# franioli/icepy4d

Measured on AMD Instinct MI355X. Metric: matched stereo image-pairs/sec (4096 kpts, 1080p), higher is better.
Workload: dtype f32

## Files before the change

### icepy4d_amd/_lib.py

```python
from __future__ import annotations

import ctypes as C
import os
import subprocess
from typing import Optional

_HERE = os.path.dirname(os.path.abspath(__file__))
CSRC = os.path.join(_HERE, "csrc")
LIB_PATH = os.environ.get("ICEMATCH_LIB") or os.path.join(CSRC, "libicematch.so")

_lib: Optional[C.CDLL] = None


class IcematchError(RuntimeError):

    def __init__(self, what: str, rc: int, message: str):
        super().__init__(f"{what} failed ({rc}): {message}")
        self.what, self.rc = what, rc


class LightGlueConf(C.Structure):
    _fields_ = [("depth_confidence", C.c_double), ("width_confidence", C.c_double),
                ("filter_threshold", C.c_double), ("n_layers", C.c_int), ("pruning_min_kpts", C.c_int)]


class SuperGlueConf(C.Structure):
    _fields_ = [("sinkhorn_iterations", C.c_int), ("match_threshold", C.c_double), ("n_layers", C.c_int)]


_P = C.c_void_p
_I = C.c_int
_F = C.c_float
_D = C.c_double
_L = C.c_longlong

SIGNATURES = {
    "im_version": [],
    "im_ctx_create": [_I, C.POINTER(_P)],
    "im_ctx_destroy": [_P],
    "im_last_error": [_P],
    "im_ctx_reserve": [_P, _I, _I, _I, _I],
    "im_profile_begin": [_P],
    "im_profile_end": [_P, C.c_char_p, C.c_size_t],
    "im_set_tensor": [_P, C.c_char_p, C.c_char_p, _P, C.c_size_t],
    "im_finalize_weights": [_P, C.c_char_p],
    "im_superpoint_forward": [_P, _P, _I, _I, _I, _I, _I, _F, _I, _I, _I, _P, _P, _P, _P, _P],
    "im_superpoint_candidates": [_P, _I, _P, _P],
    "im_lightglue_forward": [_P, _P, _P, _P, _P, C.POINTER(LightGlueConf), _P, _P, _P, _P, _P],
    "im_lightglue_forward_pairs": [_P, _I, _P, _P, _P, _P, C.POINTER(LightGlueConf), _P, _P, _P, _P, _P],
    "im_pack_records": [_P, _I, _P, _P, _P, _P, _I, _P, _P, _P],
    "im_superglue_forward": [_P, _P, _P, _P, _P, _P, C.POINTER(SuperGlueConf), _P, _P, _P, _P],
    "im_pack_record": [_P, _P, _P, _P, _P, _I, _P, _P],
    "im_debug_read": [_P, C.c_char_p, _P, C.c_size_t, _P],
    "im_debug_clock_probe": [_P, _I, _P, _P],
    "im_debug_guard_failures": [],
    "im_debug_guard_selftest": [_P, _P],
    "im_debug_guards_check": [_P, _P],
    "im_pyr_down": [_P, _P, _P, _I, _I, _I, _I, _P],
    "im_pyr_up": [_P, _P, _P, _I, _I, _I, _I, _P],
    "im_gemm_nt": [_P, _P, _P, _P, _P, _I, _I, _I, _F, _I, _P],
    "im_ffn_fused": [_P, _I, _P, _P, _P, _P, _P, _P, _P, _P, _I, _I, _P, _P],
    "im_conv3x3": [_P, _P, _P, _P, _P, _I, _I, _I, _I, _I, _I, _I, _P],
    "im_conv3x3_winograd": [_P, _P, _P, _P, _P, _I, _I, _I, _I, _I, _I, _I, _P],
    "im_flash_attn": [_P, _P, _P, _P, _P, _P, _I, _I, _I, _I, _F, _P],
    "im_nms": [_P, _P, _P, _I, _I, _I, _I, _P],
    "im_select_topk": [_P, _P, _I, _I, _I, _I, _F, _I, _P, _P, _P, _P],
    "im_sample_descriptors": [_P, _P, _I, _I, _I, _P, _P, _P, _P],
    "im_assign_from_sim": [_P, _P, _I, _I, _I, _P, _P, _F, _P, _P, _P, _P, _P],
    "im_log_optimal_transport": [_P, _P, _I, _I, _I, _F, _I, _P, _P],
    "im_merge_tile_matches": [_P, _I, _I, _P, _P, _P, _P, _P, _P, _P, _P, _P, _P, _P, _P],
    "im_gather_rows": [_P, _P, _I, _P, _I, _P, _P],
    "im_ransac_fundamental": [_P, _P, _P, _I, _I, C.c_double, C.c_uint, _P, _P, _P, _P],
    "im_ransac_essential": [_P, _P, _P, _I, _I, C.c_double, C.c_uint, _P, _P, _P, _P],
    "im_triangulate_linear": [_P, _P, _P, _P, _P, _I, _P, _P],
    "im_forient": [_P, _P, _I, _I, _I, _I, _P, _P],
    "im_template_match_oc": [_P, _P, _I, _I, _P, _I, _I, _I, _P, _P, _I, _I, _I, _I, _P, _P],
    "im_dsm_round": [_P, _P, _L, _F, _P, _P, _P, _P, _P, _P],
    "im_dsm_group_mean": [_P, _P, _P, _P, _P, _P, _P, _L, _P, _P, _P, _P, _P],
    "im_dsm_rasterize": [_P, _P, _P, _P, _P, _P, _L, _P, _P, _I, _P, _I, _D, _D, _D, _D, _D, _P, _P],
    "im_project_colors": [_P, _P, _L, _L, _P, _L, _L, _P, _L, _L, _I, _I, _I, _P, _P, _I, _I, _I, _P, _I, _P, _P, _P, _P],
    "im_undistort_points": [_P, _P, _L, _P, _P, _P],
    "im_triangulate_iterative": [_P, _P, _P, _I, _L, _P, _P, _P, _P, _D, _I, _P, _P, _P, _P, _P],
    "im_triangulate_table": [_P, _P, _I, _I, _P, _I, _I, _D, _I, _L, _P, _P, _P, _P, _P, _P],
    "im_binned_lds_capacity": [],
    "im_binned_cells": [_P, _P, _L, _I, _P, _P, _P, _P, _P, _I, _P, _P],
    "im_binned_stats": [_P, _P, _P, _L, _I, _L, _P, _I, _P, _P, _P],
    "im_tracked_points": [_P, _P, _P, _L, _P, _I, _P, _P, _P, _L, _P, _P, _P, _I, _P, _P, _P, _P, _P],
    "im_undistort_image": [_P, _P, _I, _I, _I, _I, _P, _P, _P],
    "im_warp_perspective": [_P, _P, _I, _I, _I, _I, _P, _I, _I, _P, _P],
    "im_knn_max_cells": [],
    "im_knn_cells": [_P, _P, _L, _P, _I, _I, _I, _P, _P],
    "im_knn_cell_ranges": [_P, _P, _L, _L, _P, _P],
    "im_knn_self": [_P, _P, _P, _P, _L, _P, _I, _I, _I, _I, _D, _P, _P, _P, _P, _P, _P, _P],
    "im_dod_chunk": [],
    "im_dod_max_cells": [],
    "im_dod_max_batch_cells": [],
    "im_dod_bounds": [_P, _P, _P, _I, _I, _P, _P, _P],
    "im_dod_keys": [_P, _P, _P, _I, _P, _I, _I, _D, _P, _P, _P, _P],
    "im_dod_reduce": [_P, _P, _P, _I, _P, _I, _I, _D, _P, _P, _P, _P, _P, _P],
    "im_crop_polygon": [_P, _P, _L, _I, _I, _P, _I, _I, _P, _P, _P, _P],
}


def build(force: bool = False) -> str:
    if force:
        subprocess.run(["make", "-C", CSRC, "clean"], check=True, capture_output=True)
    r = subprocess.run(["make", "-C", CSRC, "-j8"], capture_output=True, text=True)
    if r.returncode != 0:
        raise RuntimeError(f"building libicematch.so failed:\n{r.stdout[-4000:]}\n{r.stderr[-4000:]}")
    return LIB_PATH


def load() -> C.CDLL:
    global _lib
# ... 58 lines not shown
```

### icepy4d_amd/csrc/block.h

```cpp
#pragma once
#include "ctx.h"

namespace im {

struct BlockFfn {
    int act = 0;
    const float* w0 = nullptr; const float* w0p = nullptr;
    const float* b0 = nullptr;
    const float* ln_g = nullptr; const float* ln_b = nullptr;
    const float* w3 = nullptr; const float* w3p = nullptr;
    const float* b3 = nullptr;
    const char* name_fused = nullptr; const char* name_ffn0 = nullptr; const char* name_ffn3 = nullptr;
};

int launch_block_proj(im_ctx* ctx, hipStream_t s, const char* name, const GemmArgs& g, const float* wp_layers, int layer);

int launch_block_tail(im_ctx* ctx, hipStream_t s, const AttnArgs& at, const BlockFfn& f, const GemmArgs& base, float* x);

}
```

### icepy4d_amd/csrc/block.hip

```cpp
#include "block.h"

#include "lg_misc.h"
#include "workspace.h"

namespace im {

int launch_block_proj(im_ctx* ctx, hipStream_t s, const char* name, const GemmArgs& g, const float* wp_layers, int layer) {
    if (env_is_1("IM_PROJ_TILED")) {
        IM_LAUNCH(ctx, name, s, launch_gemm(g, s));
        return 0;
    }
    GemmArgs r = g;
    r.wp = reinterpret_cast<const unsigned char*>(wp_layers) + (size_t)layer * g.N * 256 * 6;
    IM_LAUNCH(ctx, name, s, launch_proj_rows(r, s));
    return 0;
}

int launch_block_tail(im_ctx* ctx, hipStream_t s, const AttnArgs& at, const BlockFfn& f, const GemmArgs& base, float* x) {
    Workspace* ws = ctx->ws;
    const long xb = (long)base.m_max * 256, hb = (long)base.m_max * 512;
    IM_LAUNCH(ctx, "attn_kv_planes", s, launch_attn_planes(at, s));
    IM_LAUNCH(ctx, at.cross ? "flash_attn_cross" : "flash_attn_self", s, launch_flash_attn(at, s));
    static const bool unfused = env_is_1("IM_FFN_UNFUSED");
    if (!unfused) {
        FfnArgs a;
        a.act = f.act; a.x = x; a.x_bstride = xb; a.att = at.out; a.att_bstride = xb;
        a.w0p = f.w0p; a.b0 = f.b0; a.ln_g = f.ln_g; a.ln_b = f.ln_b; a.w3p = f.w3p; a.b3 = f.b3;
        a.m_max = base.m_max; a.batch = base.batch; a.m_ptr = base.m_ptr; a.active = base.active; a.pstride = base.pstride;
        IM_LAUNCH(ctx, f.name_fused, s, launch_ffn_fused(a, s));
        return 0;
    }
    {
        GemmArgs g = base;
        g.A = x; g.a_bstride = xb; g.lda = 256; g.A1 = at.out; g.a1_bstride = xb; g.lda1 = 256; g.ksplit = 256;
        g.W = f.w0; g.ldw = 512; g.bias = f.b0; g.N = 512; g.K = 512;
        g.C = ws->h; g.c_bstride = hb; g.ldc = 512; g.epi = f.act == 1 ? EPI_BIAS_RELU : EPI_BIAS;
        IM_LAUNCH(ctx, f.name_ffn0, s, launch_gemm(g, s));
    }
    if (f.act == 0)
        IM_LAUNCH(ctx, "lg_layernorm_gelu", s, launch_layernorm_gelu(ws->h, hb, ws->st, base.batch, base.m_max, f.ln_g, f.ln_b, s));
    {
        GemmArgs g = base;
        g.A = ws->h; g.a_bstride = hb; g.lda = 512; g.W = f.w3; g.ldw = 512; g.bias = f.b3; g.N = 256; g.K = 512;
        g.C = x; g.c_bstride = xb; g.ldc = 256; g.R = x; g.r_bstride = xb; g.ldr = 256; g.epi = EPI_BIAS_RESID;
        IM_LAUNCH(ctx, f.name_ffn3, s, launch_gemm(g, s));
    }
    return 0;
}

}
```

### icepy4d_amd/csrc/capi.hip

```cpp
#include "ctx.h"
#include "lg_misc.h"
#include "sp_post.h"
#include "workspace.h"

#include <algorithm>
#include <cstdio>
#include <cstdlib>
#include <cstring>

using namespace im;

template <int N, typename F>
static hipError_t with_uploads(const float* const (&src)[N], const size_t (&sizes)[N], hipStream_t st, F&& launch) {
    float* d[N] = {};
    hipError_t e = hipSuccess;
    for (int i = 0; i < N && e == hipSuccess; ++i) {
        e = hipMalloc(&d[i], sizes[i] * sizeof(float));
        if (e == hipSuccess) e = hipMemcpy(d[i], src[i], sizes[i] * sizeof(float), hipMemcpyHostToDevice);
    }
    if (e == hipSuccess) e = launch(d);
    const hipError_t e2 = hipStreamSynchronize(st);
    for (int i = 0; i < N; ++i) hipFree(d[i]);
    return e != hipSuccess ? e : e2;
}
// ... 186 lines not shown
        IM_GROW(ctx, ctx->grow(ctx->scratch.clock[1], bytes, "clock_probe_convolution"), -22, "im_debug_clock_probe: allocation failed");
        IM_HIP(ctx, hipMemsetAsync(ctx->scratch.clock[0].p, 0, bytes, s));
        IM_HIP(ctx, hipMemsetAsync(ctx->scratch.clock[1].p, 0, bytes, s));
        IM_HIP(ctx, hipStreamSynchronize(s));
        ctx->clock_armed = true;
        return 0;
    }
    if (!ctx->scratch.clock[0].p || !h_out) return ctx->fail(-51, "im_debug_clock_probe: not armed");
    std::vector<unsigned long long> h((size_t)CLOCK_PROBE_SLOTS * 2);
    const void* src[2] = {ctx->scratch.clock[0].p, ctx->scratch.clock[1].p};
    for (int c = 0; c < 2; ++c) {
        IM_HIP(ctx, hipMemcpyAsync(h.data(), src[c], bytes, hipMemcpyDeviceToHost, s));
        IM_HIP(ctx, hipStreamSynchronize(s));
        std::vector<double> mhz;
        for (int i = 0; i < CLOCK_PROBE_SLOTS; ++i)
            if (h[2 * i + 1] > 0) mhz.push_back(100.0 * (double)h[2 * i] / (double)h[2 * i + 1]);
        std::sort(mhz.begin(), mhz.end());
        h_out[2 * c] = mhz.empty() ? 0.0 : mhz[mhz.size() / 2];
        h_out[2 * c + 1] = (double)mhz.size();
    }
    if (arm == 0) ctx->clock_armed = false;
    return 0;
}

int im_gemm_nt(im_ctx* ctx, const float* d_a, const float* d_w, const float* d_bias, float* d_c, int m, int n, int k,
               float alpha, int big_tile, void* stream) {
    IM_CHECK_CTX(ctx);
    GemmArgs g;
    g.A = d_a; g.lda = k; g.W = d_w; g.ldw = k; g.bias = d_bias; g.N = n; g.K = k; g.m_max = m;
    g.C = d_c; g.ldc = n; g.alpha = alpha; g.epi = EPI_BIAS; g.big_tile = big_tile & 1; g.bx = (big_tile >> 1) & 1;
    IM_HIP(ctx, launch_gemm(g, (hipStream_t)stream));
    return 0;
}

int im_ffn_fused(im_ctx* ctx, int act, float* d_x, const float* d_att, const float* h_w0, const float* h_b0, const float* h_ln_g,
                   const float* h_ln_b, const float* h_w3, const float* h_b3, int n_images, int n_rows, const int32_t* d_n, void* stream) {
    IM_CHECK_CTX(ctx);
    if (n_images < 1 || n_rows < 1 || act < 0 || act > 1 || (act == 0 && (!h_ln_g || !h_ln_b))) return ctx->fail(-12, "im_ffn_fused: bad arguments");
    if (act == 1) h_ln_g = h_ln_b = h_b0;
    const std::vector<float> p0 = pack_frag_weights(h_w0, 512, 512), p3 = pack_frag_weights(h_w3, 256, 512);
    const size_t sizes[6] = {p0.size(), 512, 512, 512, p3.size(), 256};
    const float* src[6] = {p0.data(), h_b0, h_ln_g, h_ln_b, p3.data(), h_b3};
    hipStream_t st = (hipStream_t)stream;
    IM_HIP(ctx, with_uploads(src, sizes, st, [&](float* const* d) {
        FfnArgs f;
        f.act = act; f.x = d_x; f.x_bstride = (long)n_rows * 256; f.att = d_att; f.att_bstride = (long)n_rows * 256;
        f.w0p = d[0]; f.b0 = d[1]; f.ln_g = d[2]; f.ln_b = d[3]; f.w3p = d[4]; f.b3 = d[5];
        f.m_max = n_rows; f.batch = n_images; f.m_ptr = d_n; f.pstride = 2;
        return ctx->timed("ffn_fused", st, [&] { return launch_ffn_fused(f, st); });
    }));
    return 0;
}

static int conv3x3_entry(im_ctx* ctx, bool wino, const float* d_in, const float* h_weight, const float* h_bias, float* d_out,
                         int b, int h, int w, int cin, int cout, int relu, int pool, void* stream) {
    IM_CHECK_CTX(ctx);
    if (cin % 16 || cout % 64) return ctx->fail(-10, "im_conv3x3: cin %% 16 and cout %% 64 must be 0");
    std::vector<float> packed = wino ? pack_conv3x3_wino(h_weight, cout, cin) : pack_conv3x3(h_weight, cout, cin);
    std::vector<float> planes = wino ? pack_conv3x3_wino_bx(h_weight, cout, cin) : std::vector<float>(1);
    const size_t sizes[3] = {packed.size(), (size_t)cout, planes.size()};
    const float* src[3] = {packed.data(), h_bias, planes.data()};
    hipStream_t st = (hipStream_t)stream;
    IM_HIP(ctx, with_uploads(src, sizes, st, [&](float* const* d) {
        ConvArgs a;
        a.in = d_in; a.w = d[0]; a.bias = d[1]; a.out = d_out; a.B = b; a.H = h; a.W = w; a.Cin = cin; a.Cout = cout;
        a.relu = relu; a.pool = pool;
        if (wino) a.wx = d[2];
        return ctx->timed(wino ? "conv_wino" : "conv_direct", st, [&] { return wino ? launch_conv3x3_wino(a, st) : launch_conv3x3(a, st); });
    }));
    return 0;
}

int im_conv3x3(im_ctx* ctx, const float* d_in, const float* h_weight, const float* h_bias, float* d_out, int b, int h,
               int w, int cin, int cout, int relu, int pool, void* stream) {
    return conv3x3_entry(ctx, false, d_in, h_weight, h_bias, d_out, b, h, w, cin, cout, relu, pool, stream);
}

int im_conv3x3_winograd(im_ctx* ctx, const float* d_in, const float* h_weight, const float* h_bias, float* d_out, int b,
                        int h, int w, int cin, int cout, int relu, int pool, void* stream) {
    return conv3x3_entry(ctx, true, d_in, h_weight, h_bias, d_out, b, h, w, cin, cout, relu, pool, stream);
}

int im_flash_attn(im_ctx* ctx, const float* d_q, const float* d_k, const float* d_v, float* d_out, const int32_t* d_n,
                  int n_max, int batch, int heads, int cross, float scale, void* stream) {
    IM_CHECK_CTX(ctx);
    AttnArgs a;
    a.q = d_q; a.k = d_k; a.v = d_v; a.hstride = (long)n_max * 64; a.bstride = a.hstride * heads;
    a.out = d_out; a.ldo = heads * 64; a.out_bstride = (long)n_max * a.ldo;
    a.n_ptr = d_n; a.n_max = n_max; a.batch = batch; a.heads = heads; a.cross = cross & 1; a.f32_form = (cross >> 1) & 1; a.scale = scale;
    im_ctx::StageScratch& sc = ctx->scratch;
    const bool wants_planes = !(cross & 4) && !a.f32_form;
    IM_GROW(ctx, ctx->grow(sc.attn_part, attn_part_floats(n_max, batch, heads) * sizeof(float), "stage_attn_part"), -11, "im_flash_attn: out of device memory");
    IM_GROW(ctx, ctx->grow(sc.attn_cnt, attn_counter_ints(n_max, batch, heads) * sizeof(int), "stage_attn_cnt", true), -11, "im_flash_attn: out of device memory");
    if (wants_planes) IM_GROW(ctx, ctx->grow(sc.attn_planes, attn_planes_bytes(n_max, batch, heads), "stage_attn_planes"), -11, "im_flash_attn: out of device memory");
    a.part = sc.attn_part.as<float>(); a.counters = sc.attn_cnt.as<int>(); a.planes = wants_planes ? sc.attn_planes.as<unsigned char>() : nullptr;
    IM_HIP(ctx, launch_attn_planes(a, (hipStream_t)stream));
    IM_HIP(ctx, launch_flash_attn(a, (hipStream_t)stream));
    IM_GUARD_CHECK(ctx, (hipStream_t)stream, "im_flash_attn");
    return 0;
}

int im_nms(im_ctx* ctx, const float* d_scores, float* d_out, int n_images, int h, int w, int radius, void* stream) {
    IM_CHECK_CTX(ctx);
    Workspace* ws = ctx->ws;
    if (!ws || (long)n_images * h * w > (long)ws->smap_floats)
        return ctx->fail(-41, "im_nms: exceeds the reserved workspace");
// ... 52 lines not shown
```

### icepy4d_amd/csrc/gemm.hip

```cpp
#include "bf16x3.h"
#include "common.h"
#include "kernels.h"

namespace im {

template <int BM, int BN, int BK, int EPI, bool BX>
__global__ __launch_bounds__(256) void gemm_nt_kernel(GemmArgs a) {
    constexpr int LDS_LD = BK + 4;
    constexpr int WM = BM / 2, WN = BN / 2;
    constexpr int MB = WM / 32, NB = WN / 32;
    constexpr int F4 = BK / 4;
    constexpr int A_IT = BM * F4 / 256, B_IT = BN * F4 / 256;
    constexpr int XS = BK * 2 + 16, XPA = BM * XS, XPB = BN * XS;
    __shared__ __attribute__((aligned(16))) float smem[BX ? 3 * (XPA + XPB) / 4 : (BM + BN) * LDS_LD];
    float* sA = smem;
    float* sB = smem + BM * LDS_LD;
    unsigned char* const xA = reinterpret_cast<unsigned char*>(smem);
    unsigned char* const xB = xA + 3 * XPA;

    const int gm = (a.m_max + BM - 1) / BM;
    const int z = blockIdx.y;
    const int pair = a.pair_batched ? z : (z >> 1);
    if (a.active && a.active[pair * a.pstride] == 0) return;
    const int M = a.m_ptr ? a.m_ptr[a.pair_batched ? z * a.pstride : (z >> 1) * a.pstride + (z & 1)] : a.m_max;
// ... 277 lines not shown
    {                                                                                                                \
        const unsigned char* ap = psm + c * PS + ((kc_) * 16 + hh * 8) * 2;                                          \
        const u32x4 ah = *reinterpret_cast<const u32x4*>(ap), am = *reinterpret_cast<const u32x4*>(ap + PLANE),   \
                     al = *reinterpret_cast<const u32x4*>(ap + 2 * PLANE);                                          \
        acc = mfma_bf(ah, b_[2], acc);                                                                              \
        acc = mfma_bf(al, b_[0], acc);                                                                              \
        acc = mfma_bf(am, b_[1], acc);                                                                              \
        acc = mfma_bf(ah, b_[1], acc);                                                                              \
        acc = mfma_bf(am, b_[0], acc);                                                                              \
        acc = mfma_bf(ah, b_[0], acc);                                                                              \
    }
#pragma unroll 1
    for (int j = 0; j < TILES; ++j) {
        const int tile = j * 8 + wave;
        f32x16 acc;
#pragma unroll
        for (int r = 0; r < 16; ++r) acc[r] = 0.f;
#pragma unroll 1
        for (int kc = 0; kc < 16; kc += 4) {
            const int s_ = j * 16 + kc;
            PR_LOAD(b3, s_ + 3)
            __builtin_amdgcn_sched_barrier(0);
            PR_SIX(b0, kc)
            __builtin_amdgcn_sched_barrier(0);
            PR_LOAD(b0, s_ + 4)
            __builtin_amdgcn_sched_barrier(0);
            PR_SIX(b1, kc + 1)
            __builtin_amdgcn_sched_barrier(0);
            PR_LOAD(b1, s_ + 5)
            __builtin_amdgcn_sched_barrier(0);
            PR_SIX(b2, kc + 2)
            __builtin_amdgcn_sched_barrier(0);
            PR_LOAD(b2, s_ + 6)
            __builtin_amdgcn_sched_barrier(0);
            PR_SIX(b3, kc + 3)
            __builtin_amdgcn_sched_barrier(0);
        }
        P_STAMP(2 + 2 * j)
        const int colbase = tile * 32;
        const int col = colbase + c;
        const float bv = a.bias ? a.bias[col] : 0.f;
        const unsigned rowl = m0 + 4 * hh;
        const int which = colbase >> 8, hd = colbase & 255;
        float* dst = a.q;
        if constexpr (EPI == EPI_QKV_ROPE) dst = which == 0 ? a.q : (which == 1 ? a.k : a.v);
        if constexpr (EPI == EPI_HEADS_QV) dst = which ? a.v : a.q;
        const __amdgpu_buffer_rsrc_t rD = make_rsrc(dst + (long)z * a.head_bstride + (long)(hd >> 6) * a.head_stride, (unsigned)M * 256u);
        const int d = (hd & 63) + c;
        const unsigned vo = (rowl * 64 + d) * 4u;
        float scale = a.alpha;
        if constexpr (EPI == EPI_QKV_ROPE) scale = 1.f;
        if constexpr (EPI == EPI_HEADS_QV) scale = which ? 1.f : a.alpha;
        const bool rope = EPI == EPI_QKV_ROPE && which < 2 && a.cs;
        if (rope) {
            const __amdgpu_buffer_rsrc_t rCs = make_rsrc(a.cs + (long)z * a.enc_bstride, (unsigned)M * 128u);
            const __amdgpu_buffer_rsrc_t rSn = make_rsrc(a.sn + (long)z * a.enc_bstride, (unsigned)M * 128u);
            const unsigned ve = (rowl * 32 + (d >> 1)) * 4u;
#pragma unroll
            for (int r = 0; r < 16; ++r) {
                const unsigned so = ((r & 3) + 8 * (r >> 2)) * 128u;
                const float cs = __uint_as_float(__builtin_amdgcn_raw_buffer_load_b32(rCs, ve, so, 0));
                const float sn = __uint_as_float(__builtin_amdgcn_raw_buffer_load_b32(rSn, ve, so, 0));
                const float val = acc[r] + bv;
                const float partner = __shfl_xor(val, 1);
                const float outv = (d & 1) ? (val * cs) + (partner * sn) : (val * cs) + ((-partner) * sn);
                __builtin_amdgcn_raw_buffer_store_b32(__float_as_uint(outv), rD, vo, ((r & 3) + 8 * (r >> 2)) * 256u, 0);
            }
        } else {
#pragma unroll
            for (int r = 0; r < 16; ++r)
                __builtin_amdgcn_raw_buffer_store_b32(__float_as_uint(scale * (acc[r] + bv)), rD, vo, ((r & 3) + 8 * (r >> 2)) * 256u, 0);
        }
        P_STAMP(3 + 2 * j)
    }
#undef PR_LOAD
#undef PR_SIX
}

template <int EPI, int TILES>
static hipError_t launch_proj_rows_t(const GemmArgs& a, hipStream_t s) {
    const dim3 grid((a.m_max + pr::BM - 1) / pr::BM, a.batch), block(pr::NT);
    return launch_dyn_lds<proj_rows_kernel<EPI, TILES>>(grid, block, pr::LDS_BYTES, s, a);
}

hipError_t launch_proj_rows(const GemmArgs& a, hipStream_t s) {
    if (!a.wp || a.K != 256 || a.lda != 256 || a.A1 || a.sel || a.w_bstride || a.n_ptr || a.pair_batched) return hipErrorInvalidValue;
    if (a.m_max <= 0 || a.batch <= 0) return hipSuccess;
    if (a.epi == EPI_QKV_ROPE && a.N == 768) return launch_proj_rows_t<EPI_QKV_ROPE, 3>(a, s);
    if (a.epi == EPI_HEADS_QV && a.N == 512) return launch_proj_rows_t<EPI_HEADS_QV, 2>(a, s);
    return hipErrorInvalidValue;
}

hipError_t launch_gemm(const GemmArgs& a, hipStream_t s) {
    if (a.K % 32 != 0 || (a.A1 && a.ksplit % 64 != 0)) return hipErrorInvalidValue;
    const int bm = a.big_tile ? 128 : 64, bn = bm;
    dim3 grid(((a.N + bn - 1) / bn) * ((a.m_max + bm - 1) / bm), a.batch), block(256);
    if (grid.x == 0) return hipSuccess;
#define IM_GEMM_CASE(E)                                                                  \
    case E:                                                                              \
        if (a.bx) {                                                                      \
            if (a.big_tile) hipLaunchKernelGGL((gemm_nt_kernel<128, 128, 32, E, true>), grid, block, 0, s, a);   \
            else hipLaunchKernelGGL((gemm_nt_kernel<64, 64, 32, E, true>), grid, block, 0, s, a);               \
        } else {                                                                         \
            if (a.big_tile) hipLaunchKernelGGL((gemm_nt_kernel<128, 128, 32, E, false>), grid, block, 0, s, a);  \
            else hipLaunchKernelGGL((gemm_nt_kernel<64, 64, 32, E, false>), grid, block, 0, s, a);              \
        }                                                                                \
        break;
    switch (a.epi) {
        IM_GEMM_CASE(EPI_BIAS)
        IM_GEMM_CASE(EPI_BIAS_RESID)
        IM_GEMM_CASE(EPI_HEADS)
        IM_GEMM_CASE(EPI_QKV_ROPE)
        IM_GEMM_CASE(EPI_BIAS_RELU)
        IM_GEMM_CASE(EPI_HEADS_QV)
        default: return hipErrorInvalidValue;
    }
#undef IM_GEMM_CASE
    return hipGetLastError();
}

}
```

### icepy4d_amd/csrc/kernels.h

```cpp
#pragma once
#include <hip/hip_runtime.h>
#include <stdint.h>
#include <cstdlib>
#include <vector>

#include "carve.h"
#include "common.h"

namespace im {

inline bool env_is_1(const char* name) {
    const char* e = getenv(name);
    return e && e[0] == '1';
}
inline int env_int(const char* name) {
    const char* e = getenv(name);
    return e ? atoi(e) : 0;
}

inline hipError_t current_device(int* dev) {
    if (hipError_t e = hipGetDevice(dev); e != hipSuccess) return e;
    return (*dev < 0 || *dev >= IM_MAX_DEVICES) ? hipErrorInvalidDevice : hipSuccess;
}
inline hipError_t device_cu_count(int* n) {
// ... 12 lines not shown
    int dev = 0;
    if (hipError_t e = current_device(&dev); e != hipSuccess) return e;
    if (bytes > have[dev]) {
        if (hipError_t e = hipFuncSetAttribute(reinterpret_cast<const void*>(Kernel), hipFuncAttributeMaxDynamicSharedMemorySize, (int)bytes); e != hipSuccess) return e;
        have[dev] = bytes;
    }
    return hipSuccess;
}
template <auto Kernel, typename... Args>
hipError_t launch_dyn_lds(dim3 grid, dim3 block, size_t lds_bytes, hipStream_t s, const Args&... args) {
    if (hipError_t e = optin_dyn_lds<Kernel>(lds_bytes); e != hipSuccess) return e;
    hipLaunchKernelGGL(Kernel, grid, block, lds_bytes, s, args...);
    return hipGetLastError();
}

template <typename K, typename... Args>
hipError_t launch(K kernel, dim3 blocks, int threads, size_t lds_bytes, hipStream_t s, Args... args) {
    hipLaunchKernelGGL(kernel, blocks, dim3(threads), lds_bytes, s, args...);
    return hipGetLastError();
}

enum GemmEpi {
    EPI_BIAS = 0,
    EPI_BIAS_RESID = 1,
    EPI_HEADS = 2,
    EPI_QKV_ROPE = 3,
    EPI_BIAS_RELU = 4,
    EPI_HEADS_QV = 5,
};

struct GemmArgs {
    const float* A = nullptr;  long a_bstride = 0;  int lda = 0;
    const float* A1 = nullptr; long a1_bstride = 0; int lda1 = 0; int ksplit = 0;
    const float* W = nullptr;  int ldw = 0; long w_bstride = 0;
    const float* bias = nullptr;
    const int* sel = nullptr; long w_sel_stride = 0; long bias_sel_stride = 0;
    int N = 0, K = 0;
    int m_max = 0;
    const int* m_ptr = nullptr;
    const int* n_ptr = nullptr;
    const int* active = nullptr;
    int pstride = 2;
    int pair_batched = 0;
    int batch = 1;
    float alpha = 1.f;
    float* C = nullptr; long c_bstride = 0; int ldc = 0;
    const float* R = nullptr; long r_bstride = 0; int ldr = 0;
    float* q = nullptr; float* k = nullptr; float* v = nullptr; long head_bstride = 0; long head_stride = 0;
    const float* cs = nullptr; const float* sn = nullptr; long enc_bstride = 0;
    int epi = EPI_BIAS;
    int big_tile = 0;
    int bx = 0;
    const void* wp = nullptr;
};
hipError_t launch_gemm(const GemmArgs& a, hipStream_t s);
hipError_t launch_proj_rows(const GemmArgs& a, hipStream_t s);

struct FfnArgs {
    int act = 0;
    float* x = nullptr; long x_bstride = 0;
    const float* att = nullptr; long att_bstride = 0;
    const float* w0p = nullptr; const float* b0 = nullptr;
    const float* ln_g = nullptr; const float* ln_b = nullptr;
    const float* w3p = nullptr; const float* b3 = nullptr;
    int m_max = 0; int batch = 1;
    const int* m_ptr = nullptr;
    const int* active = nullptr;
    int pstride = 2;
};
hipError_t launch_ffn_fused(const FfnArgs& a, hipStream_t s);
std::vector<float> pack_frag_weights(const float* w, int n, int k);

struct AttnArgs {
    const float* q = nullptr; const float* k = nullptr; const float* v = nullptr;
    long bstride = 0; long hstride = 0;
    float* out = nullptr; long out_bstride = 0; int ldo = 256;
    const int* n_ptr = nullptr;
    int pstride = 2;
    int n_max = 0; int batch = 2; int heads = 4; int cross = 0;
    float scale = 1.f;
    const int* active = nullptr;
    float* part = nullptr;
    int* counters = nullptr;
    void* planes = nullptr;
    int f32_form = 0;
    unsigned long long* clock = nullptr;
};
static constexpr int CLOCK_PROBE_SLOTS = 4096;
static constexpr int ATTN_MAX_SPLIT = 4;
inline size_t attn_part_floats(int n_max, int batch, int heads) { return (size_t)ATTN_MAX_SPLIT * batch * heads * n_max * 66; }
inline size_t attn_planes_bytes(int n_max, int batch, int heads) { return (size_t)2 * batch * heads * n_max * 384; }
inline size_t attn_counter_ints(int n_max, int batch, int heads) { return (size_t)batch * heads * ((n_max + 127) / 128); }
bool attn_f32_form(const AttnArgs& a);
hipError_t launch_flash_attn(const AttnArgs& a, hipStream_t s);
hipError_t launch_attn_planes(const AttnArgs& a, hipStream_t s);
hipError_t launch_flash_attn_bx(const AttnArgs& a, hipStream_t s);

struct ConvArgs {
    const float* in = nullptr;
    const float* w = nullptr;
    const float* bias = nullptr;
    float* out = nullptr;
    int B = 1, H = 0, W = 0, Cin = 0, Cout = 0;
    int pool = 0;
    int relu = 1;
    const uint8_t* img = nullptr;
// ... 17 lines not shown
```

### icepy4d_amd/csrc/lightglue.hip

```cpp
#include "block.h"
#include "lg_misc.h"
#include "workspace.h"

using namespace im;

static constexpr int ST_INTS = (int)(sizeof(LGState) / sizeof(int));

static int lg_block(im_ctx* ctx, hipStream_t s, int NI, int layer, bool cross, float* x, const float* cs, const float* sn) {
    Workspace* ws = ctx->ws;
    const LightGlueW& W = ctx->lg;
    const int K = ctx->max_kpts;
    const long xb = (long)K * 256;
    const int* n_ptr = ws->st->n;
    const int* active = &ws->st->active;
    GemmArgs base;
    base.m_max = K; base.m_ptr = n_ptr; base.active = active; base.pstride = ST_INTS; base.batch = NI; base.bx = 1;
    AttnArgs at;
    at.q = ws->q; at.k = cross ? ws->q : ws->k; at.v = ws->v; at.hstride = (long)K * 64; at.bstride = (long)K * 256;
    at.out = ws->att; at.out_bstride = xb; at.ldo = 256; at.n_ptr = n_ptr; at.pstride = ST_INTS; at.n_max = K; at.batch = NI; at.heads = 4;
    at.cross = cross ? 1 : 0; at.active = active; at.part = ws->attn_part; at.counters = ws->attn_cnt; at.planes = ws->attn_planes; at.clock = ctx->clock_of(0);
    GemmArgs g = base;
    g.A = x; g.a_bstride = xb; g.lda = 256; g.ldw = 256; g.K = 256;
    g.q = ws->q; g.v = ws->v; g.head_bstride = (long)K * 256; g.head_stride = (long)K * 64; g.big_tile = NI >= 4;
    if (!cross) {
        g.W = W.qkv_w + (long)layer * 768 * 256; g.bias = W.qkv_b + (long)layer * 768; g.N = 768; g.epi = EPI_QKV_ROPE;
        g.k = ws->k; g.cs = cs; g.sn = sn; g.enc_bstride = (long)K * 32;
        if (int rc = launch_block_proj(ctx, s, "lg_qkv_rope_gemm", g, W.qkv_wp, layer)) return rc;
        at.scale = 0.125f;
    } else {
        g.W = W.cqv_w + (long)layer * 512 * 256; g.bias = W.cqv_b + (long)layer * 512; g.N = 512; g.epi = EPI_HEADS_QV;
        g.alpha = (float)0.35355339059327373;
        if (int rc = launch_block_proj(ctx, s, "lg_proj_gemm", g, W.cqv_wp, layer)) return rc;
        at.scale = 1.f;
    }
    const LightGlueW::Ffn& F = cross ? W.cross_ffn : W.self_ffn;
    BlockFfn f;
    f.w0 = F.w0 + (long)layer * 512 * 512; f.w0p = F.w0p + (long)layer * 512 * 512 * 3 / 2; f.b0 = F.b0 + (long)layer * 512;
    f.ln_g = F.ln_g + (long)layer * 512; f.ln_b = F.ln_b + (long)layer * 512;
    f.w3 = F.w3 + (long)layer * 256 * 512; f.w3p = F.w3p + (long)layer * 256 * 512 * 3 / 2; f.b3 = F.b3 + (long)layer * 256;
    f.name_fused = "lg_ffn_fused"; f.name_ffn0 = "lg_ffn0_gemm"; f.name_ffn3 = "lg_ffn3_gemm";
    return launch_block_tail(ctx, s, at, f, base, x);
}

static int lightglue_forward(im_ctx* ctx, int n_pairs, const float* d_kpts, const float* d_desc, const int32_t* d_n, const float* h_size,
                             const im_lightglue_conf* conf, int32_t* d_matches, float* d_mscores, int32_t* d_prune, int32_t* d_info,
                             void* stream) {
    IM_CHECK_CTX(ctx);
    if (!ctx->lg.ready) return ctx->fail(-50, "im_lightglue_forward: weights not finalized");
    Workspace* ws = ctx->ws;
    if (!ws) return ctx->fail(-51, "im_lightglue_forward: call im_ctx_reserve first");
    if (n_pairs < 1 || n_pairs > ws->n_pairs || n_pairs > 64)
        return ctx->fail(-53, "im_lightglue_forward: %d pairs, the workspace was reserved for %d (max_images / 2)", n_pairs, ws->n_pairs);
    hipStream_t s = (hipStream_t)stream;
    const LightGlueW& W = ctx->lg;
    const int K = ctx->max_kpts;
    const int L = conf->n_layers;
    const int NP = n_pairs, NI = 2 * n_pairs;
    if (L < 1 || L > 9) return ctx->fail(-52, "im_lightglue_forward: n_layers must be 1..9");
    const bool do_stop = conf->depth_confidence > 0, do_prune = conf->width_confidence > 0;
    const long xb = (long)K * 256, eb = (long)K * 32;
    LGState* st = ws->st;

    IM_HIP(ctx, launch_lg_init(st, NI, d_n, ws->ind[0], ws->prune, K, K, d_matches, d_mscores, K, s));
    IM_HIP(ctx, hipMemcpyAsync(ws->x[0], d_desc, sizeof(float) * NI * xb, hipMemcpyDeviceToDevice, s));
    IM_HIP(ctx, launch_posenc(d_kpts, (long)K * 2, st, NI, K, W.wr, h_size, ws->cs[0], ws->sn[0], eb, s));
    int cur = 0;
    for (int i = 0; i < L; ++i) {
        int rc = lg_block(ctx, s, NI, i, false, ws->x[cur], ws->cs[cur], ws->sn[cur]);
        if (rc) return rc;
        rc = lg_block(ctx, s, NI, i, true, ws->x[cur], ws->cs[cur], ws->sn[cur]);
        if (rc) return rc;
        if (i == L - 1) break;
        if (!do_stop && !do_prune) continue;
        IM_LAUNCH(ctx, "lg_adapt", s, launch_rowdot(ws->x[cur], xb, st, NI, K, do_stop ? W.tc_w + (long)i * 256 : nullptr, W.tc_b + i, 1,
                                  do_prune ? W.ma_w + (long)i * 256 : nullptr, W.ma_b + i, nullptr, ws->conf, ws->msc, K,
                                  W.thr[i], do_stop ? i : -1, 1, s));
        const float keep_thr = (float)(1.0 - (double)conf->width_confidence);
        IM_LAUNCH(ctx, "lg_adapt", s, launch_stop_prune(st, NP, i, do_stop, do_prune, (float)conf->depth_confidence, keep_thr, W.thr[i], ws->conf,
                                                      ws->msc, K, ws->ind[cur], ws->ind[1 - cur], ws->keep_idx, ws->prune, K,
                                                      conf->pruning_min_kpts, s));
        if (do_prune) {
            IM_LAUNCH(ctx, "lg_adapt", s, launch_gather_rows(st, NI, K, ws->keep_idx, K, ws->x[cur], ws->x[1 - cur], xb, ws->cs[cur], ws->cs[1 - cur],
                                                           ws->sn[cur], ws->sn[1 - cur], eb, do_stop ? i : -1, (float)conf->depth_confidence, s));
            cur = 1 - cur;
        }
    }
    ctx->dbg_cur = cur;
    IM_HIP(ctx, launch_lg_select_layer(st, NP, L, ws->sel, d_info, s));
    {
        GemmArgs g;
        g.m_max = K; g.m_ptr = st->n; g.pstride = ST_INTS; g.batch = NI; g.bx = 1;
        g.A = ws->x[cur]; g.a_bstride = xb; g.lda = 256; g.W = W.fp_w; g.ldw = 256; g.bias = W.fp_b;
        g.sel = ws->sel; g.w_sel_stride = 65536; g.bias_sel_stride = 256; g.N = 256; g.K = 256;
        g.C = ws->md; g.c_bstride = xb; g.ldc = 256; g.alpha = 0.25f;
// ... 59 lines not shown
```

### include/icematch.h

```cpp
#ifndef ICEMATCH_H
#define ICEMATCH_H

#include <stddef.h>
#include <stdint.h>

#ifdef __cplusplus
extern "C" {
#endif

typedef struct im_ctx im_ctx;

int im_version(void);
int im_ctx_create(int device, im_ctx** out);
void im_ctx_destroy(im_ctx* ctx);
const char* im_last_error(im_ctx* ctx);
int im_ctx_reserve(im_ctx* ctx, int max_h, int max_w, int max_images, int max_kpts);

int im_profile_begin(im_ctx* ctx);
int im_profile_end(im_ctx* ctx, char* buf, size_t cap);

int im_set_tensor(im_ctx* ctx, const char* model, const char* key, const float* h_data, size_t numel);
int im_finalize_weights(im_ctx* ctx, const char* model);

int im_superpoint_forward(im_ctx* ctx, const uint8_t* d_img, int n_images, int h, int w, int channels,
                          int nms_radius, float threshold, int border, int max_kpts, int flavour,
                          float* d_kpts, float* d_scores, float* d_desc, int32_t* d_n, void* stream);
int im_superpoint_candidates(im_ctx* ctx, int n_images, int32_t* h_counts, void* stream);

typedef struct {
    double depth_confidence;
    double width_confidence;
    double filter_threshold;
    int n_layers;
    int pruning_min_kpts;
} im_lightglue_conf;
int im_lightglue_forward(im_ctx* ctx, const float* d_kpts, const float* d_desc, const int32_t* d_n,
                         const float* h_size, const im_lightglue_conf* conf,
                         int32_t* d_matches, float* d_mscores, int32_t* d_prune, int32_t* d_info, void* stream);

int im_lightglue_forward_pairs(im_ctx* ctx, int n_pairs, const float* d_kpts, const float* d_desc, const int32_t* d_n,
                               const float* h_size, const im_lightglue_conf* conf, int32_t* d_matches, float* d_mscores,
                               int32_t* d_prune, int32_t* d_info, void* stream);

typedef struct {
    int sinkhorn_iterations;
    double match_threshold;
    int n_layers;
} im_superglue_conf;
int im_superglue_forward(im_ctx* ctx, const float* d_kpts, const float* d_scores, const float* d_desc,
                         const int32_t* d_n, const float* h_shape, const im_superglue_conf* conf,
                         int32_t* d_matches, float* d_mscores, int32_t* d_info, void* stream);

int im_pack_record(im_ctx* ctx, const int32_t* d_n, const int32_t* d_matches0, const float* d_mscores0,
                   const int32_t* d_info, int epoch, int32_t* d_record, void* stream);
int im_pack_records(im_ctx* ctx, int n_pairs, const int32_t* d_n, const int32_t* d_matches, const float* d_mscores,
                    const int32_t* d_info, int first_epoch, int32_t* d_records, const float* d_kpts, void* stream);
int im_debug_read(im_ctx* ctx, const char* name, float* d_dst, size_t nfloats, void* stream);
int im_debug_clock_probe(im_ctx* ctx, int arm, double* h_out, void* stream);
int im_debug_guard_failures(void);
int im_debug_guard_selftest(im_ctx* ctx, void* stream);
int im_debug_guards_check(im_ctx* ctx, void* stream);

int im_gemm_nt(im_ctx* ctx, const float* d_a, const float* d_w, const float* d_bias, float* d_c,
               int m, int n, int k, float alpha, int big_tile, void* stream);
int im_ffn_fused(im_ctx* ctx, int act, float* d_x, const float* d_att, const float* h_w0, const float* h_b0, const float* h_ln_g,
                   const float* h_ln_b, const float* h_w3, const float* h_b3, int n_images, int n_rows, const int32_t* d_n, void* stream);
int im_conv3x3(im_ctx* ctx, const float* d_in, const float* h_weight, const float* h_bias, float* d_out,
               int b, int h, int w, int cin, int cout, int relu, int pool, void* stream);
int im_conv3x3_winograd(im_ctx* ctx, const float* d_in, const float* h_weight, const float* h_bias, float* d_out,
                        int b, int h, int w, int cin, int cout, int relu, int pool, void* stream);
int im_flash_attn(im_ctx* ctx, const float* d_q, const float* d_k, const float* d_v, float* d_out,
                  const int32_t* d_n, int n_max, int batch, int heads, int cross, float scale, void* stream);
int im_nms(im_ctx* ctx, const float* d_scores, float* d_out, int n_images, int h, int w, int radius, void* stream);
int im_select_topk(im_ctx* ctx, const float* d_nms, int n_images, int h, int w, int border, float threshold,
                   int max_kpts, float* d_kpts, float* d_scores, int32_t* d_n, void* stream);
int im_sample_descriptors(im_ctx* ctx, const float* d_dense_raw, int n_images, int hc, int wc,
                          const float* d_kpts, const int32_t* d_n, float* d_desc, void* stream);
int im_assign_from_sim(im_ctx* ctx, const float* d_sim, int m, int n, int ld, const float* d_z0, const float* d_z1,
                       float threshold, int32_t* d_m0, int32_t* d_m1, float* d_ms0, float* d_ms1, void* stream);
int im_log_optimal_transport(im_ctx* ctx, const float* d_scores, int m, int n, int ld, float bin_score, int iters,
                             float* d_out, void* stream);

int im_pyr_down(im_ctx* ctx, const uint8_t* d_in, uint8_t* d_out, int n_images, int h, int w, int channels, void* stream);
int im_pyr_up(im_ctx* ctx, const uint8_t* d_in, uint8_t* d_out, int n_images, int h, int w, int channels, void* stream);

int im_merge_tile_matches(im_ctx* ctx, int n_pairs, int max_kpts, const int32_t* d_matches, const int32_t* d_slots, const float* d_off,
                          const float* h_origin, const float* d_kp_bank, const int32_t* d_n_bank, int32_t* d_count, int32_t* d_idx0,
                          int32_t* d_idx1, float* d_kp0, float* d_kp1, void* stream);
int im_gather_rows(im_ctx* ctx, const float* d_src, int row_floats, const int32_t* d_idx, int n, float* d_dst, void* stream);

int im_ransac_fundamental(im_ctx* ctx, const float* d_p0, const float* d_p1, int n, int n_hyp, double threshold,
                          unsigned int seed, double* d_F, uint8_t* d_mask, int32_t* d_info, void* stream);

int im_ransac_essential(im_ctx* ctx, const float* d_x0, const float* d_x1, int n, int n_hyp, double threshold,
                        unsigned int seed, double* d_E, uint8_t* d_mask, int32_t* d_info, void* stream);

int im_triangulate_linear(im_ctx* ctx, const double* h_P0, const double* h_P1, const double* d_x0, const double* d_x1, int n,
                          double* d_X, void* stream);

int im_forient(im_ctx* ctx, const void* d_img, int dtype, int n_images, int h, int w, float* d_out, void* stream);
int im_template_match_oc(im_ctx* ctx, const float* d_a, int ha, int wa, const float* d_b, int n_b, int hb, int wb, const double* d_pairs,
                         const int32_t* d_bidx, int n_pairs, int T, int S, int conj_b, double* d_out, void* stream);

int im_dsm_round(im_ctx* ctx, const double* d_pts, long long n, float step, float* d_xr, float* d_yr, long long* d_xykey,
                 long long* d_ykey, long long* d_zkey, void* stream);
int im_dsm_group_mean(im_ctx* ctx, const double* d_pts, const float* d_xr, const float* d_yr, const long long* d_xykey,
                      const long long* d_perm_b, const long long* d_perm_c, long long n, float* d_bx, float* d_by, float* d_bz,
                      long long* d_n_groups, void* stream);
int im_dsm_rasterize(im_ctx* ctx, const float* d_bx, const float* d_by, const float* d_bz, const int32_t* d_simplices,
                     const double* d_transform, long long n_simplices, const double* h_bounds, const double* d_xq, int nx,
                     const double* d_yq, int ny, double x0, double dx, double y0, double dy, double fill, double* d_z, void* stream);
int im_project_colors(im_ctx* ctx, const double* d_x, long long sxr, long long sxc, const double* d_y, long long syr, long long syc,
                      const double* d_z, long long szr, long long szc, int rows, int cols, int cells, const double* h_cam,
                      const unsigned char* d_img, int h, int w, int cin, const int32_t* h_chmap, int cout, float* d_proj,
                      double* d_col, unsigned char* d_ortho, void* stream);

int im_undistort_points(im_ctx* ctx, const float* d_pts, long long n, const double* h_cam, float* d_out, void* stream);
int im_triangulate_iterative(im_ctx* ctx, const void* d_u1, const void* d_u2, int f64, long long n, const double* h_P1,
                             const double* h_P2, const double* h_cam1, const double* h_cam2, double tolerance, int max_solves,
// ... 45 lines not shown
```

Baseline: 169.0.

## Write K/V attention planes directly from projection GEMM epilogue

The QKV/QV projection epilogue now splits K and V outputs into the three-way precision planes that attention consumes, writing them directly. The separate attn_kv_planes kernel then becomes unnecessary for LightGlue layers and is skipped. This removes one kernel launch and a full read and rewrite of K/V per layer, at the cost of extra stores, DPP shuffles and register pressure in the GEMM epilogue. A test entry point, im_proj_planes, is added to compare both paths.

```diff
diff --git a/icepy4d_amd/_lib.py b/icepy4d_amd/_lib.py
--- a/icepy4d_amd/_lib.py
+++ b/icepy4d_amd/_lib.py
@@ -60,6 +60,7 @@
     "im_pyr_up": [_P, _P, _P, _I, _I, _I, _I, _P],
     "im_gemm_nt": [_P, _P, _P, _P, _P, _I, _I, _I, _F, _I, _P],
     "im_ffn_fused": [_P, _I, _P, _P, _P, _P, _P, _P, _P, _P, _I, _I, _P, _P],
+    "im_proj_planes": [_P, _I, _P, _P, _P, _P, _P, _P, _P, _I, _I, _F, _I, _P, _P, _P],
     "im_conv3x3": [_P, _P, _P, _P, _P, _I, _I, _I, _I, _I, _I, _I, _P],
     "im_conv3x3_winograd": [_P, _P, _P, _P, _P, _I, _I, _I, _I, _I, _I, _I, _P],
     "im_flash_attn": [_P, _P, _P, _P, _P, _P, _I, _I, _I, _I, _F, _P],
diff --git a/icepy4d_amd/csrc/block.h b/icepy4d_amd/csrc/block.h
--- a/icepy4d_amd/csrc/block.h
+++ b/icepy4d_amd/csrc/block.h
@@ -15,6 +15,8 @@
 
 int launch_block_proj(im_ctx* ctx, hipStream_t s, const char* name, const GemmArgs& g, const float* wp_layers, int layer);
 
-int launch_block_tail(im_ctx* ctx, hipStream_t s, const AttnArgs& at, const BlockFfn& f, const GemmArgs& base, float* x);
+bool block_proj_writes_planes(const AttnArgs& at);
+
+int launch_block_tail(im_ctx* ctx, hipStream_t s, const AttnArgs& at, const BlockFfn& f, const GemmArgs& base, float* x, bool planes_filled = false);
 
 }
diff --git a/icepy4d_amd/csrc/block.hip b/icepy4d_amd/csrc/block.hip
--- a/icepy4d_amd/csrc/block.hip
+++ b/icepy4d_amd/csrc/block.hip
@@ -16,10 +16,14 @@
     return 0;
 }
 
-int launch_block_tail(im_ctx* ctx, hipStream_t s, const AttnArgs& at, const BlockFfn& f, const GemmArgs& base, float* x) {
+bool block_proj_writes_planes(const AttnArgs& at) {
+    return at.planes && !attn_f32_form(at) && !env_is_1("IM_PROJ_TILED") && !env_is_1("IM_KV_PLANE_PASS");
+}
+
+int launch_block_tail(im_ctx* ctx, hipStream_t s, const AttnArgs& at, const BlockFfn& f, const GemmArgs& base, float* x, bool planes_filled) {
     Workspace* ws = ctx->ws;
     const long xb = (long)base.m_max * 256, hb = (long)base.m_max * 512;
-    IM_LAUNCH(ctx, "attn_kv_planes", s, launch_attn_planes(at, s));
+    if (!planes_filled) IM_LAUNCH(ctx, "attn_kv_planes", s, launch_attn_planes(at, s));
     IM_LAUNCH(ctx, at.cross ? "flash_attn_cross" : "flash_attn_self", s, launch_flash_attn(at, s));
     static const bool unfused = env_is_1("IM_FFN_UNFUSED");
     if (!unfused) {
diff --git a/icepy4d_amd/csrc/capi.hip b/icepy4d_amd/csrc/capi.hip
--- a/icepy4d_amd/csrc/capi.hip
+++ b/icepy4d_amd/csrc/capi.hip
@@ -262,6 +262,41 @@
     return 0;
 }
 
+int im_proj_planes(im_ctx* ctx, int cross, const float* d_x, const float* h_w, const float* h_bias, const float* d_cos, const float* d_sin,
+                   const int32_t* d_n, const int32_t* d_active, int n_images, int n_rows, float alpha, int plane_pass, float* d_q, void* d_planes,
+                   void* stream) {
+    IM_CHECK_CTX(ctx);
+    if (n_images < 2 || n_images % 2 || n_rows < 1 || !d_x || !h_w || !h_bias || !d_q || !d_planes || (!cross && (!d_cos || !d_sin)))
+        return ctx->fail(-12, "im_proj_planes: bad arguments");
+    if (plane_pass && attn_f32_form(AttnArgs())) return ctx->fail(-12, "im_proj_planes: IM_ATTN_F32 is set, there is no plane pass in this process");
+    const int N = cross ? 512 : 768;
+    const std::vector<float> wp = pack_frag_weights(h_w, N, 256);
+    hipStream_t st = (hipStream_t)stream;
+    const size_t img = (size_t)n_rows * 256;
+    float* d_kv = nullptr;
+    if (plane_pass) IM_HIP(ctx, hipMalloc(&d_kv, 2 * n_images * img * sizeof(float)));
+    const size_t sizes[2] = {wp.size(), (size_t)N};
+    const float* src[2] = {wp.data(), h_bias};
+    const hipError_t e = with_uploads(src, sizes, st, [&](float* const* d) {
+        GemmArgs g;
+        g.A = d_x; g.a_bstride = (long)img; g.lda = 256; g.ldw = 256; g.K = 256; g.N = N; g.wp = d[0]; g.bias = d[1];
+        g.m_max = n_rows; g.m_ptr = d_n; g.active = d_active; g.pstride = 2; g.batch = n_images; g.bx = 1;
+        g.q = d_q; g.k = d_kv; g.v = d_kv ? d_kv + n_images * img : nullptr; g.head_bstride = (long)img; g.head_stride = (long)n_rows * 64;
+        g.epi = cross ? EPI_HEADS_QV : EPI_QKV_ROPE; g.alpha = cross ? alpha : 1.f;
+        if (!cross) { g.cs = d_cos; g.sn = d_sin; g.enc_bstride = (long)n_rows * 32; }
+        if (!plane_pass) g.planes = d_planes;
+        if (hipError_t le = launch_proj_rows(g, st); le != hipSuccess || !plane_pass) return le;
+        AttnArgs a;
+        a.k = cross ? d_q : g.k; a.v = g.v; a.hstride = g.head_stride; a.bstride = g.head_bstride;
+        a.n_ptr = d_n; a.active = d_active; a.pstride = 2; a.n_max = n_rows; a.batch = n_images; a.heads = 4; a.planes = d_planes;
+        return launch_attn_planes(a, st);
+    });
+    hipFree(d_kv);
+    IM_HIP(ctx, e);
+    IM_GUARD_CHECK(ctx, st, "im_proj_planes");
+    return 0;
+}
+
 static int conv3x3_entry(im_ctx* ctx, bool wino, const float* d_in, const float* h_weight, const float* h_bias, float* d_out,
                          int b, int h, int w, int cin, int cout, int relu, int pool, void* stream) {
     IM_CHECK_CTX(ctx);
diff --git a/icepy4d_amd/csrc/gemm.hip b/icepy4d_amd/csrc/gemm.hip
--- a/icepy4d_amd/csrc/gemm.hip
+++ b/icepy4d_amd/csrc/gemm.hip
@@ -353,10 +353,26 @@
         if constexpr (EPI == EPI_QKV_ROPE) scale = 1.f;
         if constexpr (EPI == EPI_HEADS_QV) scale = which ? 1.f : a.alpha;
         const bool rope = EPI == EPI_QKV_ROPE && which < 2 && a.cs;
+        const bool to_planes = a.planes && (EPI == EPI_HEADS_QV || which != 0);
+        const bool to_f32 = !a.planes || which == 0;
+        const int kv = EPI == EPI_QKV_ROPE ? which - 1 : which;
+        const __amdgpu_buffer_rsrc_t rP = make_rsrc(reinterpret_cast<unsigned char*>(a.planes) +
+            (to_planes ? ((long)kv * a.batch * a.head_bstride + (long)z * a.head_bstride + (long)(hd >> 6) * a.head_stride) * 6 : 0L), to_planes ? (unsigned)M * 384u : 0u);
+        const unsigned vp = ((rowl + (d & 1)) * 384u) + (unsigned)(d & ~1) * 2u;
+        auto store_planes = [&](int i, float u0, float u1) {
+            const float got = __uint_as_float(__builtin_amdgcn_update_dpp(0u, __float_as_uint((d & 1) ? u0 : u1), 0xB1, 0xF, 0xF, true));
+            unsigned h, m, l;
+            split2((d & 1) ? got : u0, (d & 1) ? u1 : got, h, m, l);
+            const unsigned so = (((2 * i) & 3) + 8 * ((2 * i) >> 2)) * 384u;
+            __builtin_amdgcn_raw_buffer_store_b32(h, rP, vp, so, 0);
+            __builtin_amdgcn_raw_buffer_store_b32(m, rP, vp, so + 128u, 0);
+            __builtin_amdgcn_raw_buffer_store_b32(l, rP, vp, so + 256u, 0);
+        };
         if (rope) {
             const __amdgpu_buffer_rsrc_t rCs = make_rsrc(a.cs + (long)z * a.enc_bstride, (unsigned)M * 128u);
             const __amdgpu_buffer_rsrc_t rSn = make_rsrc(a.sn + (long)z * a.enc_bstride, (unsigned)M * 128u);
             const unsigned ve = (rowl * 32 + (d >> 1)) * 4u;
+            float ov[16];
 #pragma unroll
             for (int r = 0; r < 16; ++r) {
                 const unsigned so = ((r & 3) + 8 * (r >> 2)) * 128u;
@@ -365,12 +381,23 @@
                 const float val = acc[r] + bv;
                 const float partner = __shfl_xor(val, 1);
                 const float outv = (d & 1) ? (val * cs) + (partner * sn) : (val * cs) + ((-partner) * sn);
-                __builtin_amdgcn_raw_buffer_store_b32(__float_as_uint(outv), rD, vo, ((r & 3) + 8 * (r >> 2)) * 256u, 0);
+                ov[r] = outv;
+                if (to_f32) __builtin_amdgcn_raw_buffer_store_b32(__float_as_uint(outv), rD, vo, ((r & 3) + 8 * (r >> 2)) * 256u, 0);
+            }
+            if (to_planes) {
+#pragma unroll
+                for (int i = 0; i < 8; ++i) store_planes(i, ov[2 * i], ov[2 * i + 1]);
             }
         } else {
-#pragma unroll
-            for (int r = 0; r < 16; ++r)
-                __builtin_amdgcn_raw_buffer_store_b32(__float_as_uint(scale * (acc[r] + bv)), rD, vo, ((r & 3) + 8 * (r >> 2)) * 256u, 0);
+            if (to_f32) {
+#pragma unroll
+                for (int r = 0; r < 16; ++r)
+                    __builtin_amdgcn_raw_buffer_store_b32(__float_as_uint(scale * (acc[r] + bv)), rD, vo, ((r & 3) + 8 * (r >> 2)) * 256u, 0);
+            }
+            if (to_planes) {
+#pragma unroll
+                for (int i = 0; i < 8; ++i) store_planes(i, scale * (acc[2 * i] + bv), scale * (acc[2 * i + 1] + bv));
+            }
         }
         P_STAMP(3 + 2 * j)
     }
@@ -386,6 +413,7 @@
 
 hipError_t launch_proj_rows(const GemmArgs& a, hipStream_t s) {
     if (!a.wp || a.K != 256 || a.lda != 256 || a.A1 || a.sel || a.w_bstride || a.n_ptr || a.pair_batched) return hipErrorInvalidValue;
+    if (a.planes && (a.head_stride != (long)a.m_max * 64 || a.head_bstride != 4 * a.head_stride)) return hipErrorInvalidValue;
     if (a.m_max <= 0 || a.batch <= 0) return hipSuccess;
     if (a.epi == EPI_QKV_ROPE && a.N == 768) return launch_proj_rows_t<EPI_QKV_ROPE, 3>(a, s);
     if (a.epi == EPI_HEADS_QV && a.N == 512) return launch_proj_rows_t<EPI_HEADS_QV, 2>(a, s);
@@ -393,7 +421,7 @@
 }
 
 hipError_t launch_gemm(const GemmArgs& a, hipStream_t s) {
-    if (a.K % 32 != 0 || (a.A1 && a.ksplit % 64 != 0)) return hipErrorInvalidValue;
+    if (a.K % 32 != 0 || (a.A1 && a.ksplit % 64 != 0) || a.planes) return hipErrorInvalidValue;
     const int bm = a.big_tile ? 128 : 64, bn = bm;
     dim3 grid(((a.N + bn - 1) / bn) * ((a.m_max + bm - 1) / bm), a.batch), block(256);
     if (grid.x == 0) return hipSuccess;
diff --git a/icepy4d_amd/csrc/kernels.h b/icepy4d_amd/csrc/kernels.h
--- a/icepy4d_amd/csrc/kernels.h
+++ b/icepy4d_amd/csrc/kernels.h
@@ -88,6 +88,7 @@
     int big_tile = 0;
     int bx = 0;
     const void* wp = nullptr;
+    void* planes = nullptr;
 };
 hipError_t launch_gemm(const GemmArgs& a, hipStream_t s);
 hipError_t launch_proj_rows(const GemmArgs& a, hipStream_t s);
diff --git a/icepy4d_amd/csrc/lightglue.hip b/icepy4d_amd/csrc/lightglue.hip
--- a/icepy4d_amd/csrc/lightglue.hip
+++ b/icepy4d_amd/csrc/lightglue.hip
@@ -22,6 +22,8 @@
     GemmArgs g = base;
     g.A = x; g.a_bstride = xb; g.lda = 256; g.ldw = 256; g.K = 256;
     g.q = ws->q; g.v = ws->v; g.head_bstride = (long)K * 256; g.head_stride = (long)K * 64; g.big_tile = NI >= 4;
+    const bool proj_planes = block_proj_writes_planes(at);
+    if (proj_planes) g.planes = at.planes;
     if (!cross) {
         g.W = W.qkv_w + (long)layer * 768 * 256; g.bias = W.qkv_b + (long)layer * 768; g.N = 768; g.epi = EPI_QKV_ROPE;
         g.k = ws->k; g.cs = cs; g.sn = sn; g.enc_bstride = (long)K * 32;
@@ -39,7 +41,7 @@
     f.ln_g = F.ln_g + (long)layer * 512; f.ln_b = F.ln_b + (long)layer * 512;
     f.w3 = F.w3 + (long)layer * 256 * 512; f.w3p = F.w3p + (long)layer * 256 * 512 * 3 / 2; f.b3 = F.b3 + (long)layer * 256;
     f.name_fused = "lg_ffn_fused"; f.name_ffn0 = "lg_ffn0_gemm"; f.name_ffn3 = "lg_ffn3_gemm";
-    return launch_block_tail(ctx, s, at, f, base, x);
+    return launch_block_tail(ctx, s, at, f, base, x, proj_planes);
 }
 
 static int lightglue_forward(im_ctx* ctx, int n_pairs, const float* d_kpts, const float* d_desc, const int32_t* d_n, const float* h_size,
diff --git a/include/icematch.h b/include/icematch.h
--- a/include/icematch.h
+++ b/include/icematch.h
@@ -65,6 +65,9 @@
                int m, int n, int k, float alpha, int big_tile, void* stream);
 int im_ffn_fused(im_ctx* ctx, int act, float* d_x, const float* d_att, const float* h_w0, const float* h_b0, const float* h_ln_g,
                    const float* h_ln_b, const float* h_w3, const float* h_b3, int n_images, int n_rows, const int32_t* d_n, void* stream);
+int im_proj_planes(im_ctx* ctx, int cross, const float* d_x, const float* h_w, const float* h_bias, const float* d_cos, const float* d_sin,
+                   const int32_t* d_n, const int32_t* d_active, int n_images, int n_rows, float alpha, int plane_pass, float* d_q,
+                   void* d_planes, void* stream);
 int im_conv3x3(im_ctx* ctx, const float* d_in, const float* h_weight, const float* h_bias, float* d_out,
                int b, int h, int w, int cin, int cout, int relu, int pool, void* stream);
 int im_conv3x3_winograd(im_ctx* ctx, const float* d_in, const float* h_weight, const float* h_bias, float* d_out,
```

Result: no change. 169.6 (median of 6 runs) (+0.4%).
